# buggyyang/CDC_compression

Hardware: AMD Instinct MI355X
Metric: decoded images/sec at 256x256, 500-step x-param (higher is better)
Workload: dtype f32 (f16x2 split products)

## Files before the change

cdc_compression_amd/_lib.py:

```python
import ctypes
import os
import subprocess

import numpy as np

_HERE = os.path.dirname(os.path.abspath(__file__))
LIB_PATH = os.environ.get("CDC_HIP_LIB") or os.path.join(_HERE, "libcdc_hip.so")

CDC_MEM_HOST, CDC_MEM_DEVICE = 0, 1
CDC_PRED_X, CDC_PRED_NOISE, CDC_PRED_NOISE_XTREE, CDC_PRED_V = 0, 1, 2, 3
CDC_CLIP_NONE, CDC_CLIP_ALL, CDC_CLIP_HALF = 0, 1, 2
CDC_MAX_LEVELS = 8
CDC_ELEM_F32, CDC_ELEM_U8 = 0, 1
CDC_FILL_EDGE, CDC_FILL_ZERO = 0, 1
CDC_METRIC_PSNR, CDC_METRIC_MSSSIM = 1, 2
CDC_TRACE_X0, CDC_TRACE_XT, CDC_TRACE_U8 = 1, 2, 4

_f = ctypes.POINTER(ctypes.c_float)
_i = ctypes.c_int
_vp = ctypes.c_void_p


class UnetConfig(ctypes.Structure):
    _fields_ = [("dim", ctypes.c_int32), ("channels", ctypes.c_int32),
# ... 138 lines not shown
    L.cdc_prof_name.argtypes = [_i]
    L.cdc_prof_name.restype = ctypes.c_char_p
    L.cdc_prof_get.argtypes = [H, _i, ctypes.POINTER(ctypes.c_double),
                               ctypes.POINTER(ctypes.c_int64), ctypes.POINTER(ctypes.c_double),
                               ctypes.POINTER(ctypes.c_double)]
    L.cdc_prof_reset.argtypes = [H]
    L.cdc_prof_num_ops.argtypes = [H]
    L.cdc_prof_op.argtypes = [H, _i, ctypes.POINTER(ctypes.c_char_p), ctypes.POINTER(ctypes.c_double),
                              ctypes.POINTER(ctypes.c_int64), ctypes.POINTER(ctypes.c_double)]
    L.cdc_op_conv2d.argtypes = [H, _vp, _vp, _vp, _vp] + [_i] * 9 + [_vp, _vp, _i, _vp, _vp]
    L.cdc_op_conv_transpose2d.argtypes = [H, _vp, _vp, _vp, _vp] + [_i] * 5
    L.cdc_op_chan_layernorm.argtypes = [H, _vp, _vp, _vp, _vp, _i, _i, _i]
    L.cdc_op_chan_layernorm_ex.argtypes = [H, _vp, _i, _vp, _vp, _i, _vp, _vp, _i, _vp, _vp, _vp, _i, _i, _i]
    L.cdc_op_ln_form.argtypes = [H, _i, _i, _i, _i, _i] + [ctypes.POINTER(_i)] * 4
    L.cdc_op_sum_slices.argtypes = [H, _vp, _i, _vp, _i, ctypes.c_longlong]
    L.cdc_op_linear_attention.argtypes = [H] + [_vp] * 7 + [_i] * 4
    L.cdc_op_stress.argtypes = [H, _i]
    L.cdc_op_stress_result.argtypes = [H, ctypes.POINTER(ctypes.c_int64), ctypes.POINTER(ctypes.c_int64)]
    L.cdc_probe_mfma_f16.argtypes = [_i, _i, _i, ctypes.POINTER(ctypes.c_double)]
    L.cdc_probe_hbm_copy.argtypes = [_i, ctypes.c_size_t, _i, ctypes.POINTER(ctypes.c_double)]
    _lib = L
    return L


EXPORTS = ["cdc_create", "cdc_destroy", "cdc_last_error", "cdc_version", "cdc_num_tensors",
           "cdc_tensor_info", "cdc_load_tensor", "cdc_finalize_weights", "cdc_unet_forward",
           "cdc_set_schedule", "cdc_ddim_step", "cdc_decode", "cdc_prof_enable",
           "cdc_prof_num_classes", "cdc_prof_name", "cdc_prof_get", "cdc_prof_reset",
           "cdc_op_conv2d", "cdc_op_conv_transpose2d", "cdc_op_chan_layernorm",
           "cdc_op_linear_attention", "cdc_ctxdec_create", "cdc_ctxdec_decode", "cdc_hyperdec_create",
           "cdc_hyperdec_decode", "cdc_dequantize", "cdc_bpp", "cdc_encoder_create",
           "cdc_encoder_encode", "cdc_set_arith", "cdc_get_arith", "cdc_unet_tap", "cdc_prof_num_ops", "cdc_prof_op",
           "cdc_entropy_encode", "cdc_entropy_peek", "cdc_entropy_set_limit", "cdc_entropy_decode", "cdc_get_range_faults",
           "cdc_get_nonfinite_results", "cdc_set_schedule_v", "cdc_probe_mfma_f16", "cdc_probe_hbm_copy",
           "cdc_op_stress", "cdc_op_stress_result", "cdc_enable_vbr", "cdc_set_bitrate_scale", "cdc_entropy_peek_bitrate_scale",
           "cdc_padded_size", "cdc_frame_pad", "cdc_frame_crop", "cdc_entropy_set_image_scale", "cdc_entropy_encode_image",
           "cdc_entropy_peek_image_size", "cdc_decode_seeded", "cdc_randn", "cdc_randn_host", "cdc_philox4x32_10",
           "cdc_distortion", "cdc_lpips_create", "cdc_lpips", "cdc_simple_encoder_create", "cdc_simple_ctxdec_create", "cdc_op_gdn",
           "cdc_op_gdn_workgroups", "cdc_op_chan_layernorm_ex", "cdc_op_ln_form", "cdc_op_sum_slices",
           "cdc_set_solver", "cdc_decode_solver", "cdc_solver_step", "cdc_op_solver_update", "cdc_op_ddim_update",
           "cdc_repeat_images", "cdc_decode_samples", "cdc_sample_moments", "cdc_sample_select",
           "cdc_set_trace", "cdc_trace_info", "cdc_trace_read", "cdc_op_trace_tap"]


def handle_status(handle):
    if handle is None:
        return {"arith": None, "range_faults": 0, "nonfinite_results": 0}
    L = lib()
    return {"arith": int(L.cdc_get_arith(handle)), "range_faults": int(L.cdc_get_range_faults(handle)),
            "nonfinite_results": int(L.cdc_get_nonfinite_results(handle))}


def check(handle, rc):
    if rc != 0:
        msg = lib().cdc_last_error(handle)
        msg = msg.decode() if msg else ""
        if "must be multiples of" in msg:
# ... 90 lines not shown
```

cdc_compression_amd/csrc/cdc_internal.h:

```cpp
#pragma once
#include <stdio.h>
#include <string.h>
#include <stdlib.h>
#include <hip/hip_runtime.h>
#include <map>
#include <mutex>
#include <utility>
#include <stdint.h>

#include <string>
#include <vector>

#include "conv_args.h"

extern "C" char **environ;

namespace cdc {

typedef void (*conv_kernel_fn)(const ConvArgs);
conv_kernel_fn conv_lookup_a(int MB, int NPW, int lnmode);
conv_kernel_fn conv_lookup_b(int MB, int NPW, int lnmode);
conv_kernel_fn conv_lookup_c(int MB, int NPW, int lnmode);
conv_kernel_fn conv_lookup_split(int MB, int NPW);
conv_kernel_fn conv_lookup_split2(int MB, int NPW, int lnmode, int xu = 1);
// ... 23 lines not shown
    int stride = 1;
    int uf = 0;
    int cop = 0;
    int tz = 1;
};
struct PfPlan {
    int MB, NPW, WM, WP, ring, tiles_x, tiles_y, groups; size_t lds_bytes; int lin = 0;
    int x16 = 0;
    int pf3_epv = 0, pf3_G = 0, pf3_iters = 0;
};
bool pf_make_plan(const PfShape &s, PfPlan *plan);
hipError_t pf_launch(PfArgs a, const PfPlan &plan, int B, int nz, hipStream_t st);
bool pf3_make_plan(const PfArgs &a, int B, int nz, PfPlan *plan);
hipError_t pf3_launch(PfArgs a, const PfPlan &plan, int B, hipStream_t st);
int device_cus();
struct WsPlan { int W, NPB, stride, waves, tiles, groups; size_t lds_bytes; };
struct WsArgs;
bool ws_make_plan(int Cin, int C0, int Cout, int H, int W, int B, int stride, WsPlan *plan);
hipError_t ws_launch(WsArgs a, const WsPlan &plan, hipStream_t st);
struct Ws1Plan { int NPB, waves, tiles, groups; size_t lds_bytes; };
struct Ws1Args;
bool ws1_make_plan(int Cin, int C0, int Cout, int HW, int B, bool per_image_w, Ws1Plan *plan);
hipError_t ws1_launch(Ws1Args a, const Ws1Plan &plan, hipStream_t st);
bool pw_make_plan(const PfShape &s, PfPlan *plan);
hipError_t pw_launch(PfArgs a, const PfPlan &plan, int B, hipStream_t st);
hipError_t pf_pack_launch(const float *src, long long src_bs, void *dst, long long dst_bs, int C, int H, int W, int B,
                          hipStream_t st);
hipError_t c4_pack_launch(const float *src, long long src_bs, float *dst, int C, long long HW, int B, hipStream_t st);
hipError_t pf_unpack_launch(const void *src, long long src_bs, float *dst, long long dst_bs, int C, int H, int W, int B, hipStream_t st);

// ... 228 lines not shown
```

cdc_compression_amd/csrc/cdc_planner.hip:

```cpp
#include "cdc_state.h"

namespace cdcapi {

constexpr int kKsTarget = 1024;

struct Builder {
    cdc_handle *h;
    int B;
    std::vector<void *> *pool;
    int rc = CDC_OK;
    int planB = 0;
    int pb() const { return planB > 0 ? planB : B; }
    std::vector<Op> *cur = nullptr;

    void emit(Op op) {
        op.id = (int)h->op_ms.size();
        h->op_ms.push_back(0); h->op_n.push_back(0); h->op_flops.push_back(op.flops);
        const bool hoisted = cur == &h->pre_ops;
        char buf[160];
        std::visit([&](const auto &payload) { op_label(payload, buf, sizeof buf, hoisted); }, op.p);
        if (hoisted && !strstr(buf, " HOIST") && strlen(buf) + 7 < sizeof buf) strcat(buf, " HOIST");
        h->op_label.push_back(buf);
        (cur ? cur : &h->ops)->push_back(op);
    }
// ... 1493 lines not shown
int cdc_op_ln_form(cdc_handle *h, int B, int C, int HW, int nparts, int aligned16, int *kind, int *width, int *np, int *img_major) {
    if (!h) return CDC_ERR_INVALID;
    if (B < 1 || C < 1 || HW < 1 || nparts < 1) return fail(h, CDC_ERR_INVALID, "cdc_op_ln_form: B = %d, C = %d, HW = %d, nparts = %d", B, C, HW, nparts);
    if (nparts > 1 && C > 384) return fail(h, CDC_ERR_INVALID, "cdc_op_ln_form: %d split-K slices over %d > 384 channels", nparts, C);
    LnArgs a = {};
    a.C = C; a.HW = HW; a.nparts = nparts; a.part_stride = (long long)B * C * HW;
    a.in = reinterpret_cast<const float *>((uintptr_t)(aligned16 ? 16 : 4));
    const LnForm f = ln_form(a, B);
    if (kind) *kind = f.kind;
    if (width) *width = f.width;
    if (np) *np = f.np;
    if (img_major) *img_major = f.img_major;
    return CDC_OK;
}

int cdc_op_linear_attention(cdc_handle *h, const float *x, const float *norm_g, const float *norm_b,
                            const float *w_qkv, const float *w_out, const float *b_out, float *y, int B,
                            int C, int H, int W) {
    return with_range_guard(h, [&] { return op_linear_attention_impl(h, x, norm_g, norm_b, w_qkv, w_out, b_out, y, B, C, H, W); });
}

static int op_gdn_impl(cdc_handle *h, const float *x, const float *beta, const float *gamma, float *y, int B, int C, int HW, int inverse) {
    int rc = op_ready(h);
    if (rc) return rc;
    if (!x || !beta || !gamma || !y || B < 1 || HW < 1) return fail(h, CDC_ERR_INVALID, "null/invalid argument");
    if (!gdn_supported(C)) return fail(h, CDC_ERR_UNSUPPORTED, "GDN over %d channels: the kernel takes multiples of 16 from 16 to 256", C);
    OpScope sc(h);
    Builder bd{h, B, &sc.pool};
    std::vector<float> br((size_t)C), gr((size_t)C * C);
    gdn_reparam(beta, gamma, C, br.data(), gr.data());
// ... 48 lines not shown
```

cdc_compression_amd/csrc/conv_args.h:

```cpp
#pragma once
#include <stdint.h>

namespace cdc {

constexpr int kWaveSize = 64;
constexpr int kXS = 20;

struct ConvArgs {
    const float *src0, *src1;
    long long src0_bs, src1_bs;
    int uf_c, uf_pad;
    unsigned uf_magic;
    int C0, Cin;
    int H, W;
    const float *ln_mean, *ln_rstd;
    const float *ln_g, *ln_b;
    const float *wp;
    long long w_bs, w_zs;
    const unsigned short *wsp;
    long long wsp_zs;
    long long wsp_bs;
    float acc_scale;
    int tg;
    int ipw, B;
// ... 73 lines not shown
    long long resid1_bs;
    int resid_c0;
    const void *resid_pf;
    long long rpf_bs, rpf_ps;
    int rpf_ys, rpf_zoff;
    float *stat_mean, *stat_rstd;
    const float *res3_w, *res3_x;
    long long res3_bs;
    const float *x0, *x1;
    long long x0_bs, x1_bs;
    const float *pre_mean, *pre_rstd;
    long long w_bs;
    int lin;
    int dbg;
    int *fault;
#ifdef CDC_TIMELINE
    unsigned long long *tl;
#endif
};

constexpr int kPfXS = 12;

struct ConvPlan {
    int MB, NPW, WN;
    int groups;
    int KC, nchunk;
    int lognbw, tiles_x, tiles_y, PH, PW;
    int xvec, xshift[4];
    size_t lds_bytes;
    int lnmode;
// ... 10 lines not shown
```

cdc_compression_amd/csrc/conv_inst_p.hip:

```cpp
#include <algorithm>
#include <map>
#include <string>
#include <vector>
#include <stdlib.h>

#include "cdc_internal.h"
#include "conv_pf_kernel.h"

namespace cdc {

template <int KH, int KW>
static pf_kernel_fn pf_lookup_k(int MB, int NPW, int WM, int WP) {
    if (MB == 2 && NPW == 2 && WM == 1 && WP == 4) return conv_pf_kernel<2, 2, 1, 4, KH, KW>;
    if (MB == 2 && NPW == 2 && WM == 2 && WP == 2) return conv_pf_kernel<2, 2, 2, 2, KH, KW>;
    if (MB == 2 && NPW == 2 && WM == 2 && WP == 4) return conv_pf_kernel<2, 2, 2, 4, KH, KW>;
    if (MB == 3 && NPW == 2 && WM == 2 && WP == 4) return conv_pf_kernel<3, 2, 2, 4, KH, KW>;
    if (MB == 3 && NPW == 1 && WM == 2 && WP == 4 && KH == 3) return conv_pf_kernel<3, 1, 2, 4, KH, KW>;
    if (MB == 2 && NPW == 2 && WM == 4 && WP == 2) return conv_pf_kernel<2, 2, 4, 2, KH, KW>;
    return nullptr;
}
static pf_kernel_fn pf_lookup_s2(int MB, int NPW, int WM, int WP) {
    if (MB == 2 && NPW == 1 && WM == 1 && WP == 4) return conv_pf_kernel<2, 1, 1, 4, 3, 3, 2>;
    if (MB == 2 && NPW == 2 && WM == 2 && WP == 2) return conv_pf_kernel<2, 2, 2, 2, 3, 3, 2>;
    if (MB == 3 && NPW == 1 && WM == 2 && WP == 4) return conv_pf_kernel<3, 1, 2, 4, 3, 3, 2>;
// ... 148 lines not shown
            p->groups = s.Cout / COPT;
            p->lds_bytes = std::max(patch + ring * wst, sizeof(float) * (size_t)(4 * COPT + 2 * c.WM * c.WP * c.NPW * 32));
        }
    }
    return best >= 0;
}

hipError_t pf_launch(PfArgs a, const PfPlan &p, int B, int nz, hipStream_t st) {
    if (p.pf3_epv) return pf3_launch(a, p, B, st);
    pf_kernel_fn fn = pf_lookup(p.MB, p.NPW, p.WM, p.WP, a.KH, a.KW, a.stride == 2 ? 2 : 1, a.tz == 4 ? 4 : 1);
    if (!fn) return hipErrorInvalidValue;
    if (a.tz == 4) nz = 1;
    a.lognbw = 5;
    a.dbg = 0;
    a.tiles_x = p.tiles_x; a.tiles_y = p.tiles_y; a.B = B; a.ring = p.ring;
    if (hipError_t e = ensure_dynamic_lds((const void *)fn, p.lds_bytes); e != hipSuccess) return e;
    dim3 grid((unsigned)(p.tiles_x * p.tiles_y * B), (unsigned)p.groups, (unsigned)nz);
    a.xcd_remap = (grid.x % 8 == 0 && grid.x >= 64) ? 1 : 0;
#ifdef CDC_TIMELINE
    static unsigned long long *tl_dev = nullptr;
    static std::map<std::string, int> seen;
    const size_t tl_wgs = (size_t)grid.x * grid.y * grid.z;
    char key[96];
    snprintf(key, sizeof key, "%dx%d s%d tz%d %d->%d out %dx%d", a.KH, a.KW, a.stride == 2 ? 2 : 1, a.tz == 4 ? 4 : 1, a.Cin, a.Cout, a.Ho, a.Wo);
    a.tl = nullptr;
    if (tl_wgs <= (1u << 18) && seen[key]++ < 3) {
        if (!tl_dev) hipMalloc(&tl_dev, sizeof(unsigned long long) * 16 * (1u << 18));
        hipMemsetAsync(tl_dev, 0, sizeof(unsigned long long) * 16 * tl_wgs, st);
        a.tl = tl_dev;
    }
#endif
    hipLaunchKernelGGL(fn, grid, dim3(64 * p.WM * p.WP), p.lds_bytes, st, a);
#ifdef CDC_TIMELINE
    if (a.tl) {
        hipStreamSynchronize(st);
        std::vector<unsigned long long> h(16 * tl_wgs);
        hipMemcpy(h.data(), tl_dev, h.size() * 8, hipMemcpyDeviceToHost);
        unsigned long long t0 = ~0ull, t1 = 0;
        double cat[7] = {0}, life = 0;
        std::map<unsigned long long, int> per_cu;
        std::vector<unsigned long long> starts;
        for (size_t w = 0; w < tl_wgs; ++w) {
            const unsigned long long *r = &h[w * 16];
            for (int c = 0; c < 7; ++c) cat[c] += (double)r[c];
            t0 = std::min(t0, r[7]); t1 = std::max(t1, r[8]);
            life += (double)(r[8] - r[7]);
            per_cu[(r[10] & 0xf) << 32 | (r[9] & 0xffff00)]++;
// ... 89 lines not shown
```

cdc_compression_amd/csrc/conv_pf_kernel.h:

```cpp
#pragma once
#include <type_traits>

#include "conv_split_kernel.h"

namespace cdc {


#ifndef CDC_DMA_WAIT_MARGIN
#define CDC_DMA_WAIT_MARGIN 1
#endif
#ifdef CDC_DMA_WAIT_ALL
constexpr int kVmWaitMask = 0;
#else
constexpr int kVmWaitMask = ~0;
#endif
template <int N> __device__ __forceinline__ void vm_wait() { asm volatile("s_waitcnt vmcnt(%0)" ::"n"(N & kVmWaitMask) : "memory"); }

__device__ __forceinline__ void dma16(unsigned voff, const void *sbase, unsigned lds_byte) {
    asm volatile("s_mov_b32 m0, %2\n\ts_nop 0\n\tglobal_load_lds_dwordx4 %0, %1" ::"v"(voff), "s"(sbase), "s"(lds_byte)
                 : "memory");
}

template <int N, class F> __device__ __forceinline__ void static_for(F &&f) {
    if constexpr (N > 0) {
// ... 27 lines not shown
#define CDC_PF_S2_TPS 3
#endif
#ifndef CDC_PF_TZ_MINB
#define CDC_PF_TZ_MINB 2
#endif
#ifndef CDC_PF_TZ_TPS
#define CDC_PF_TZ_TPS 2
#endif
__host__ __device__ constexpr int pf_tps(int MB, int NPW, int WM, int WP, int KH, int KW, int STR = 1, int TZ = 1) {
    if (TZ == 4) return (CDC_PF_TZ_TPS > 1 && pf_ring_tps(MB, NPW, WM, WP, KH, KW, STR, CDC_PF_TZ_TPS, TZ) >= 3) ? CDC_PF_TZ_TPS : 1;
    return (STR == 2 && CDC_PF_S2_TPS > 1 && pf_ring_tps(MB, NPW, WM, WP, KH, KW, STR, CDC_PF_S2_TPS) >= 3) ? CDC_PF_S2_TPS : 1;
}
__host__ __device__ constexpr int pf_ring(int MB, int NPW, int WM, int WP, int KH, int KW, int STR = 1, int TZ = 1) {
    return pf_ring_tps(MB, NPW, WM, WP, KH, KW, STR, pf_tps(MB, NPW, WM, WP, KH, KW, STR, TZ), TZ);
}
#ifndef CDC_PF_ABLATE
#define CDC_PF_ABLATE 0
#endif

template <int MB, int NPW, int WM, int WP, int KH, int KW, int STR = 1, int TZ = 1, int UF = 0>
__global__ void __launch_bounds__(64 * WM * WP, (KH == 1 && KW == 7) ? 3 : STR == 2 ? 1 : ((WM * WP == 8 || MB * NPW * TZ <= 4 || (TZ == 4 && MB * NPW <= 2 && CDC_PF_TZ_MINB == 2)) ? 2 : 1)) conv_pf_kernel(const PfArgs P) {
    constexpr int NW = WM * WP, NT = 64 * NW, COPT = WM * MB * 32;
    static_assert(COPT % 64 == 0 || COPT == 32, "a weight DMA instruction (64 units) must stay inside one (plane, k-half) row");
    static_assert(TZ == 1 || (TZ == 4 && KH == 2 && KW == 2 && STR == 1), "fused phases: the 2x2 phase form of the 4x4 transposed convolution");
    constexpr int NB = TZ * NPW;
    constexpr bool ACC2 = pf_acc2(MB, NB);
    constexpr int NPL = ACC2 ? 2 : 3, ROWS = 2 * NPL;
    constexpr int WI = (ROWS * COPT + 63) / 64;
    constexpr int NWV = NW - 2;
    constexpr int NWW = (WI + NWV - 1) / NWV;
    constexpr int TAPZ = KH * KW, TAPS = TAPZ * TZ;
    constexpr int NBW = 32, NBH = 1;
    constexpr int TH = WP * NPW * NBH;
    constexpr int PH = TZ == 4 ? TH + 2 : (TH - 1) * STR + KH, PW = TZ == 4 ? NBW + 2 : (NBW - 1) * STR + KW, PLANE = PH * PW;
    constexpr int NE = (PW + 1) / 2;
// ... 20 lines not shown
        unsigned hw_; asm volatile("s_getreg_b32 %0, hwreg(HW_REG_HW_ID)" : "=s"(hw_)); r_[9] = hw_; \
        unsigned xcc_; asm volatile("s_getreg_b32 %0, hwreg(HW_REG_XCC_ID)" : "=s"(xcc_)); r_[10] = xcc_; } } while (0)
#else
#define PFTL(c) do { } while (0)
#define PFTL_END() do { } while (0)
#endif
    const int tid = threadIdx.x, lane = tid & 63;
    const int wave = __builtin_amdgcn_readfirstlane(tid >> 6);
    const int wm = wave / WP, wp = wave % WP;
    const bool patch_wave = wave >= NWV;
    const int pwi = wave - NWV;
    const int z = blockIdx.z, cog = blockIdx.y;
    unsigned bid0 = blockIdx.x;
    if (P.xcd_remap) bid0 = (bid0 & 7) * (gridDim.x >> 3) + (bid0 >> 3);
    int bid = (int)bid0;
    const int tx = bid % P.tiles_x;
    bid /= P.tiles_x;
    const int ty = bid % P.tiles_y;
    const int b = bid / P.tiles_y;
    const int oy0 = ty * TH, ox0 = tx * NBW;
    const int S = P.nchunk * SPC;
    constexpr int R = pf_ring(MB, NPW, WM, WP, KH, KW, STR, TZ);
    static_assert(R >= 3, "no room for a weight ring");
    const unsigned lds0 = __builtin_amdgcn_readfirstlane((unsigned)(size_t)(const __attribute__((address_space(3))) uint4 *)smem_u);
    const unsigned wl_lds = lds0 + (unsigned)(NPB * PST) * 16u;

    const int Hp = P.H + 2, Wp = P.W + 2;
    const int iy0 = oy0 * STR - P.pad_y[z] + 1, ix0 = ox0 * STR - P.pad_x[z] + 1;
    unsigned xoff[KX];
#pragma unroll
    for (int i = 0; i < KX; ++i) {
        int e = (2 * i + (pwi & 1)) * 64 + lane;
        if (e >= NX) e = 0;
        const int q = e / PLANE, rem = e - q * PLANE;
        const int r = rem / PW, cp = rem - r * PW;
        const int c = STR == 2 ? (cp < NE ? 2 * cp : 2 * (cp - NE) + 1) : cp;
        const int iy = min(max(iy0 + r, 0), Hp - 1), ix = min(max(ix0 + c, 0), Wp - 1);
        xoff[i] = (unsigned)((q * Hp + iy) * Wp + ix) * 16u;
    }
    const long long cg_bytes = (long long)4 * Hp * Wp * 16;
    const char *s0 = reinterpret_cast<const char *>(P.src0) + (size_t)b * P.src0_bs * 16;
    const char *s1 = P.src1 ? reinterpret_cast<const char *>(P.src1) + (size_t)b * P.src1_bs * 16 : nullptr;
    const int c0_chunks = P.C0 >> 4;
    constexpr int ISSUE_TAPS = TAPS >= 9 ? 6 : (TAPS == 7 ? 5 : (TAPS >= 4 ? 2 : 1));
    constexpr int PER = (KX + ISSUE_TAPS - 1) / ISSUE_TAPS;
    auto issue_patch = [&](int chunk, auto tc) {
        constexpr int t = decltype(tc)::value;
        const char *base = chunk < c0_chunks ? s0 + (long long)chunk * cg_bytes : s1 + (long long)(chunk - c0_chunks) * cg_bytes;
        int pb = chunk;
        if constexpr (NPB == 2) pb &= 1; else pb %= 3;
        const unsigned dst = lds0 + (unsigned)(pb * PST) * 16u + (unsigned)(pwi & 1) * 1024u;
#pragma unroll
        for (int i = 0; i < KX; ++i)
            if (t < 0 || i / PER == t)
// ... 18 lines not shown
    const char *wptr = wsrc;
    int tw = 0, sw = 0;
    auto issue_w = [&]() {
        const unsigned dst = wl_lds + (unsigned)(sw * WST) * 16u;
#pragma unroll
        for (int q = 0; q < TPS; ++q)
#pragma unroll
            for (int k = 0; k < NWW; ++k) dma16(wvo[k], wptr + q * w_dt, dst + (unsigned)(q * TAPW) * 16u + wdo[k]);
        tw += TPS;
        if (tw == TAPS) { tw = 0; wptr += w_dc; }
        else if (TZ > 1 && (tw % TAPZ) == 0) wptr += w_dz;
        else wptr += TPS * w_dt;
        if (++sw == R) sw = 0;
    };

    f32x16 acc[MB][NB], acc2[ACC2 ? MB : 1][ACC2 ? NB : 1];
#pragma unroll
    for (int m = 0; m < MB; ++m)
#pragma unroll
        for (int n = 0; n < NB; ++n)
#pragma unroll
            for (int r = 0; r < 16; ++r) {
                acc[m][n][r] = 0.f;
                if constexpr (ACC2) acc2[m][n][r] = 0.f;
            }

    const int half = lane >> 5, j = lane & 31;
    const int pr = 0, pc = j;
    const uint4 *a_base = smem_u + NPB * PST + half * COPT + wm * MB * 32 + j;
    const uint4 *b_base = smem_u + (half * 2) * PLANE + (wp * NPW * STR) * PW + j;

// ... 33 lines not shown
#pragma unroll
            for (int term = 0; term < 3; ++term) {
                constexpr int PA[3] = {1, 2, 0};
                constexpr int PB[3] = {0, 1, 0};
#pragma unroll
                for (int m = 0; m < MB; ++m)
#pragma unroll
                    for (int n = 0; n < NPW; ++n)
                        acc[m][q0 + n] = __builtin_amdgcn_mfma_f32_32x32x16_f16(A[PA[term] % NPL][m], Bv[PB[term]][n], acc[m][q0 + n], 0, 0, 0);
            }
        }
    };

    PFTL(0);
    if constexpr (UF != 0) {
        if (!patch_wave)
            for (int q = 0; q < R - 1 && q < S; ++q) issue_w();
        constexpr int XW = NBW + 6;
        float *xs = reinterpret_cast<float *>(smem_u + NPB * PST + R * WST);
        {
            constexpr int NS = (UF * PH * XW + NT - 1) / NT;
            float sv[NS];
#pragma unroll
            for (int k = 0; k < NS; ++k) {
                const int i = tid + k * NT;
                const int ci = i / (PH * XW), rem = i - ci * (PH * XW), r = rem / XW, cc = rem - r * XW;
                const int iy = oy0 - 3 + r, ix = ox0 - 3 + cc;
                sv[k] = (i < UF * PH * XW && iy >= 0 && iy < P.H && ix >= 0 && ix < P.W) ? P.x0[(size_t)b * P.x0_bs + ((size_t)ci * P.H + iy) * P.W + ix] : 0.f;
            }
#pragma unroll
            for (int k = 0; k < NS; ++k)
                if (tid + k * NT < UF * PH * XW) xs[tid + k * NT] = sv[k];
// ... 5 lines not shown
#pragma unroll
            for (int ch = 0; ch < 32; ++ch) {
                if (ch < 7 * UF) split2h(xs[((ch % UF) * PH + r) * XW + c + ch / UF], hq[ch], lq[ch]);
                else { hq[ch] = (_Float16)0.f; lq[ch] = (_Float16)0.f; }
            }
#pragma unroll
            for (int q = 0; q < 4; ++q) {
                f16x8 hv, lv;
#pragma unroll
                for (int t = 0; t < 8; ++t) { hv[t] = hq[8 * q + t]; lv[t] = lq[8 * q + t]; }
                uint4 *pbuf = smem_u + (q >> 1) * PST + ((q & 1) * 2) * PLANE + px;
                pbuf[0] = __builtin_bit_cast(uint4, hv);
                pbuf[PLANE] = __builtin_bit_cast(uint4, lv);
            }
        }
    } else if (patch_wave) {
        for (int c = 0; c < LA && c < P.nchunk; ++c) issue_patch(c, std::integral_constant<int, -1>{});
    } else {
        for (int q = 0; q < R - 1 && q < S; ++q) issue_w();
    }
    PFTL(1);
    dma_wait();
    __builtin_amdgcn_s_barrier();
    PFTL(2);
    OpsA A0, A1;
    OpsB B0, B1;
    fetch(std::integral_constant<int, 0>{}, b_base, a_base, A0, B0);
    int rem = S - 1;
    int sn = 0;
    auto tap = [&](auto tc, auto tailc, int chunk, const uint4 *xb_cur, const uint4 *xb_nxt, OpsA &Ac, OpsB &Bc, OpsA &An,
                   OpsB &Bn) {
        constexpr int t = decltype(tc)::value;
        constexpr bool TAIL = decltype(tailc)::value;
        constexpr bool SEND = (t % TPS) == TPS - 1;
// ... 59 lines not shown
    } else {
        int chunk = 0;
        for (; chunk + 1 < n_main; chunk += 2) {
            chunk_body(P0{}, std::false_type{}, chunk);
            chunk_body(P1{}, std::false_type{}, chunk + 1);
        }
        for (; chunk + 1 < P.nchunk; chunk += 2) {
            chunk_body(P0{}, std::true_type{}, chunk);
            chunk_body(P1{}, std::true_type{}, chunk + 1);
        }
        if (chunk < P.nchunk) chunk_body(P0{}, std::true_type{}, chunk);
    }

    __builtin_amdgcn_s_barrier();
    PFTL(3);
    if (CDC_PF_ABLATE && (P.dbg & 256)) { PFTL_END(); return; }
    float *ep = reinterpret_cast<float *>(smem_u);
    float *red = ep + 4 * COPT;
    for (int i = tid; i < COPT; i += NT) {
        const int co = cog * COPT + i;
        const bool ok = co < P.Cout;
        ep[i] = (ok && P.bias) ? P.bias[co] : 0.f;
        ep[COPT + i] = (ok && P.ep_g) ? P.ep_g[co] : 0.f;
        ep[2 * COPT + i] = (ok && P.ep_b) ? P.ep_b[co] : 0.f;
        ep[3 * COPT + i] = (ok && P.shift) ? P.shift[(size_t)b * P.shift_bs + co] : 0.f;
    }
    __syncthreads();
    PFTL(4);
    const float inv_c = 1.0f / (float)P.Cout;
    const int cobase = cog * COPT + wm * MB * 32;
    const float *epl = ep + wm * MB * 32 + 4 * half;
    const bool ch_ok = cobase + MB * 32 <= P.Cout || COPT == 32;
    const int nvalid = P.Cout - cobase;
    if constexpr (TZ == 4) {
        if (!P.pre_add && !P.resid && !P.resid_pf && !P.res3_w && !P.relu && !P.shift && !P.stat_mean && (WM == 1 || !P.ep_g)) {
            static_assert(!ACC2, "fused phases: one accumulator set");
#pragma unroll
            for (int py = 0; py < 2; ++py)
#pragma unroll
                for (int n = 0; n < NPW; ++n) {
                    const int q0 = (py * 2) * NPW + n, q1 = q0 + NPW;
                    const int oy = oy0 + (wp * NPW + n) * NBH + pr, ox = ox0 + pc;
// ... 78 lines not shown
                                    const uint2 sh = half ? a0 : a1, sl = half ? c0 : c1;
                                    uint2 rh, rl;
                                    rh.x = __shfl_xor(sh.x, 32); rh.y = __shfl_xor(sh.y, 32);
                                    rl.x = __shfl_xor(sl.x, 32); rl.y = __shfl_xor(sl.y, 32);
                                    const uint4 uh = half ? make_uint4(rh.x, rh.y, a1.x, a1.y) : make_uint4(a0.x, a0.y, rh.x, rh.y);
                                    const uint4 ul = half ? make_uint4(rl.x, rl.y, c1.x, c1.y) : make_uint4(c0.x, c0.y, rl.x, rl.y);
                                    uint4 *pu = reinterpret_cast<uint4 *>(P.out_pf) + u0 + (long long)((cobase >> 3) + m * 4 + g) * 2 * P.pf_ps;
                                    pu[0] = uh;
                                    pu[P.pf_ps] = ul;
                                }
                        }
                    }
                    __builtin_amdgcn_sched_barrier(0);
                }
            PFTL(6);
            PFTL_END();
            return;
        }
    }
    float mean_v[NB], rinv_v[NB];
    bool valid_v[NB];
    unsigned pix_v[NB];
#pragma unroll
    for (int n = 0; n < NB; ++n) {
        const int oy = oy0 + (wp * NPW + n % NPW) * NBH + pr, ox = ox0 + pc;
        const int zn = TZ == 4 ? n / NPW : z;
        valid_v[n] = (oy < P.Ho) && (ox < P.Wo) && ch_ok;
        pix_v[n] = (unsigned)(oy * P.out_ys + ox * P.out_xs + P.out_zoff[zn]);
        const float *eq = epl;
#pragma unroll
        for (int m = 0; m < MB; ++m)
#pragma unroll
// ... 197 lines not shown
                            const uint2 a0 = __builtin_bit_cast(uint2, hv0), a1 = __builtin_bit_cast(uint2, hv1);
                            const uint2 c0 = __builtin_bit_cast(uint2, lv0), c1 = __builtin_bit_cast(uint2, lv1);
                            const uint2 sh = half ? a0 : a1, sl = half ? c0 : c1;
                            uint2 rh, rl;
                            rh.x = __shfl_xor(sh.x, 32); rh.y = __shfl_xor(sh.y, 32);
                            rl.x = __shfl_xor(sl.x, 32); rl.y = __shfl_xor(sl.y, 32);
                            const uint4 uh = half ? make_uint4(rh.x, rh.y, a1.x, a1.y) : make_uint4(a0.x, a0.y, rh.x, rh.y);
                            const uint4 ul = half ? make_uint4(rl.x, rl.y, c1.x, c1.y) : make_uint4(c0.x, c0.y, rl.x, rl.y);
                            uint4 *pu = reinterpret_cast<uint4 *>(P.out_pf) + u0 + (long long)((cobase >> 3) + m * 4 + g) * 2 * P.pf_ps;
                            pu[0] = uh;
                            pu[P.pf_ps] = ul;
                        }
                }
            }
        PFTL(6);
        PFTL_END();
        return;
    }
#pragma unroll
    for (int n = 0; n < NB; ++n) {
        if (!valid_v[n] || (CDC_PF_ABLATE && (P.dbg & 16))) continue;
        if (P.out) {
            float *op = P.out + (size_t)b * P.out_bs + pix_v[n] + (size_t)(cobase + 4 * half) * P.out_cs;
#pragma unroll
            for (int m = 0; m < MB; ++m)
#pragma unroll
                for (int r = 0; r < 16; ++r) {
                    const int ci = m * 32 + (r & 3) + 8 * (r >> 2);
                    if (COPT != 32 || ci + 4 * half < nvalid) op[(size_t)ci * P.out_cs] = acc[m][n][r];
                }
        }
        if (P.out_pf) {
            const int oy = oy0 + (wp * NPW + n % NPW) * NBH + pr, ox = ox0 + pc;
            const long long u0 = (long long)b * P.pf_bs + (long long)oy * P.pf_ys + (long long)ox * P.pf_xs + P.pf_zoff[TZ == 4 ? n / NPW : z];
#pragma unroll
            for (int m = 0; m < MB; ++m)
                pf_store_block(reinterpret_cast<uint4 *>(P.out_pf), u0 + (long long)((cobase >> 3) + m * 4) * 2 * P.pf_ps, P.pf_ps, half, acc[m][n]);
        }
    }
    PFTL(6);
    PFTL_END();
}

typedef void (*pf_kernel_fn)(const PfArgs);

}
```

cdc_compression_amd/ops.py:

```python
import ctypes

import numpy as np

from . import _lib


def _c(a):
    return None if a is None else np.ascontiguousarray(a, dtype=np.float32)


def _p(a):
    return None if a is None else a.ctypes.data


class Ops:
    def __init__(self, device=0):
        def config():
            cfg = _lib.UnetConfig()
            cfg.dim, cfg.channels, cfg.context_channels, cfg.out_dim = 32, 3, 3, 3
            cfg.n_dim_mults = 1
            cfg.dim_mults[0] = 1
            cfg.n_context_dim_mults = 1
            cfg.context_dim_mults[0] = 1
            return cfg
# ... 94 lines not shown
        return y

    def gdn(self, x, beta, gamma, inverse=False):
        x, beta, gamma = _c(x), _c(beta).reshape(-1), _c(gamma)
        B, C, H, W = x.shape
        if beta.shape != (C,) or gamma.shape != (C, C):
            raise ValueError(f"beta {beta.shape} / gamma {gamma.shape} do not belong to {C} channels")
        y = np.empty_like(x)
        _lib.check(self._h, _lib.lib().cdc_op_gdn(self._h, _p(x), _p(beta), _p(gamma), _p(y), B, C, H * W, int(bool(inverse))))
        return y

    def gdn_workgroups(self, B, HW):
        per_image, tiles = ctypes.c_int(), ctypes.c_int()
        _lib.check(self._h, _lib.lib().cdc_op_gdn_workgroups(self._h, int(B), int(HW), ctypes.byref(per_image), ctypes.byref(tiles)))
        return per_image.value, tiles.value
```

include/cdc_hip.h:

```cpp
#ifndef CDC_HIP_H
#define CDC_HIP_H

#include <stddef.h>
#include <stdint.h>

#ifdef __cplusplus
extern "C" {
#endif

typedef struct cdc_handle cdc_handle;

typedef enum {
    CDC_OK = 0,
    CDC_ERR_INVALID = -1,
    CDC_ERR_STATE = -2,
    CDC_ERR_HIP = -3,
    CDC_ERR_UNSUPPORTED = -4,
    CDC_ERR_NOMEM = -5
} cdc_status;

enum { CDC_MEM_HOST = 0, CDC_MEM_DEVICE = 1 };
enum { CDC_PRED_X = 0, CDC_PRED_NOISE = 1, CDC_PRED_NOISE_XTREE = 2, CDC_PRED_V = 3 };
enum { CDC_CLIP_NONE = 0, CDC_CLIP_ALL = 1, CDC_CLIP_HALF = 2 };
enum { CDC_MAX_LEVELS = 8 };
// ... 183 lines not shown
int cdc_prof_num_ops(cdc_handle *h);
int cdc_prof_op(cdc_handle *h, int idx, const char **label, double *ms, int64_t *launches, double *flops);


int cdc_op_conv2d(cdc_handle *h, const float *x, const float *w, const float *bias, float *y,
                  int B, int Cin, int H, int W, int Cout, int KH, int KW, int stride, int pad,
                  const float *ln_g, const float *ln_b, int relu, const float *shift,
                  const float *resid);
int cdc_op_conv_transpose2d(cdc_handle *h, const float *x, const float *w, const float *bias,
                            float *y, int B, int Cin, int H, int W, int Cout);
int cdc_op_chan_layernorm(cdc_handle *h, const float *x, const float *g, const float *b, float *y,
                          int B, int C, int HW);
int cdc_op_chan_layernorm_ex(cdc_handle *h, const float *x, int nparts, const float *g, const float *b, int relu, const float *shift,
                             const float *resid, int in_place, float *y, float *stat_mean, float *stat_rstd, int B, int C, int HW);
int cdc_op_ln_form(cdc_handle *h, int B, int C, int HW, int nparts, int aligned16, int *kind, int *width, int *np, int *img_major);
int cdc_op_sum_slices(cdc_handle *h, const float *x, int parts, float *y, int B, long long n);
int cdc_op_gdn(cdc_handle *h, const float *x, const float *beta, const float *gamma, float *y, int B, int C, int HW, int inverse);
int cdc_op_gdn_workgroups(cdc_handle *h, int B, int HW, int *per_image, int *tiles);
int cdc_op_linear_attention(cdc_handle *h, const float *x, const float *norm_g,
                            const float *norm_b, const float *w_qkv, const float *w_out,
                            const float *b_out, float *y, int B, int C, int H, int W);

int cdc_op_stress(cdc_handle *h, int repeats);
int cdc_op_stress_result(cdc_handle *h, int64_t *launches, int64_t *differing);

#ifdef __cplusplus
}
#endif
#endif
```

Before: 5.271.

## Add persistent walking form of stride-2 3x3 pf conv kernel

Adds a WALK template variant of the pf conv kernel in which each workgroup processes a contiguous range of tiles in a loop, sized to the number of resident slots. While the current tile's epilogue runs, it prefetches the next tile's patches and weights, and it reuses the bias and LN epilogue parameters across tiles. Only stride-2 3x3 shapes with two specific MB/NPW/WM/WP configs use it. It aims to cut per-workgroup launch, prologue and pipeline-fill cost, in exchange for more LDS use, a more complex kernel and possible load imbalance across workgroups.

```diff
diff --git a/cdc_compression_amd/_lib.py b/cdc_compression_amd/_lib.py
--- a/cdc_compression_amd/_lib.py
+++ b/cdc_compression_amd/_lib.py
@@ -176,6 +176,11 @@
     L.cdc_op_chan_layernorm_ex.argtypes = [H, _vp, _i, _vp, _vp, _i, _vp, _vp, _i, _vp, _vp, _vp, _i, _i, _i]
     L.cdc_op_ln_form.argtypes = [H, _i, _i, _i, _i, _i] + [ctypes.POINTER(_i)] * 4
     L.cdc_op_sum_slices.argtypes = [H, _vp, _i, _vp, _i, ctypes.c_longlong]
+    L.cdc_pf_walk_ranges.argtypes = [_i, _i, _i, _vp]
+    L.cdc_pf_walk_tile.argtypes = [_i, _i, _i, _i]
+    L.cdc_pf_walk_wgs.argtypes = [_i, _i]
+    L.cdc_pf_walk_launches.argtypes = []
+    L.cdc_pf_walk_launches.restype = ctypes.c_longlong
     L.cdc_op_linear_attention.argtypes = [H] + [_vp] * 7 + [_i] * 4
     L.cdc_op_stress.argtypes = [H, _i]
     L.cdc_op_stress_result.argtypes = [H, ctypes.POINTER(ctypes.c_int64), ctypes.POINTER(ctypes.c_int64)]
@@ -202,7 +207,8 @@
            "cdc_op_gdn_workgroups", "cdc_op_chan_layernorm_ex", "cdc_op_ln_form", "cdc_op_sum_slices",
            "cdc_set_solver", "cdc_decode_solver", "cdc_solver_step", "cdc_op_solver_update", "cdc_op_ddim_update",
            "cdc_repeat_images", "cdc_decode_samples", "cdc_sample_moments", "cdc_sample_select",
-           "cdc_set_trace", "cdc_trace_info", "cdc_trace_read", "cdc_op_trace_tap"]
+           "cdc_set_trace", "cdc_trace_info", "cdc_trace_read", "cdc_op_trace_tap",
+           "cdc_pf_walk_ranges", "cdc_pf_walk_tile", "cdc_pf_walk_wgs", "cdc_pf_walk_launches"]
 
 
 def handle_status(handle):
diff --git a/cdc_compression_amd/csrc/cdc_internal.h b/cdc_compression_amd/csrc/cdc_internal.h
--- a/cdc_compression_amd/csrc/cdc_internal.h
+++ b/cdc_compression_amd/csrc/cdc_internal.h
@@ -3,6 +3,8 @@
 #include <string.h>
 #include <stdlib.h>
 #include <hip/hip_runtime.h>
+#include <algorithm>
+#include <atomic>
 #include <map>
 #include <mutex>
 #include <utility>
@@ -61,6 +63,23 @@
 bool pf3_make_plan(const PfArgs &a, int B, int nz, PfPlan *plan);
 hipError_t pf3_launch(PfArgs a, const PfPlan &plan, int B, hipStream_t st);
 int device_cus();
+typedef void (*pf_kernel_fn_t)(const PfArgs);
+pf_kernel_fn_t pf_walk_lookup(int MB, int NPW, int WM, int WP, int KH, int KW, int stride, int tz);
+extern std::atomic<long long> g_pf_walk_launches;
+inline int pf_walk_wgs(int tiles, int slots) {
+    const int g = std::max(1, std::min(tiles, slots));
+    return g >= 64 ? g & ~7 : g;
+}
+inline int pf_walk_first(int tiles, int wgs, int wg) { return wg * (tiles / wgs) + std::min(wg, tiles % wgs); }
+inline int pf_walk_tile(int t, int tiles_x, int tiles_y, int col_major) {
+    const int per = tiles_x * tiles_y, b = t / per, ti = t % per;
+    return col_major ? b * per + (ti % tiles_y) * tiles_x + ti / tiles_y : t;
+}
+inline int pf_walk_slots(int KH, int KW, int stride, size_t lds_bytes, int yz) {
+    int per_cu = stride == 2 ? 1 : ((KH == 1 && KW == 7) ? 3 : 2);
+    if (lds_bytes) per_cu = std::max(1, std::min(per_cu, (int)(160 * 1024 / lds_bytes)));
+    return std::max(1, device_cus() * per_cu / std::max(1, yz));
+}
 struct WsPlan { int W, NPB, stride, waves, tiles, groups; size_t lds_bytes; };
 struct WsArgs;
 bool ws_make_plan(int Cin, int C0, int Cout, int H, int W, int B, int stride, WsPlan *plan);
diff --git a/cdc_compression_amd/csrc/cdc_planner.hip b/cdc_compression_amd/csrc/cdc_planner.hip
--- a/cdc_compression_amd/csrc/cdc_planner.hip
+++ b/cdc_compression_amd/csrc/cdc_planner.hip
@@ -1531,6 +1531,22 @@
     return CDC_OK;
 }
 
+int cdc_pf_walk_ranges(int tiles, int wgs_lo, int wgs_hi, int *first) {
+    if (tiles < 1 || wgs_lo < 1 || wgs_hi < wgs_lo || !first) return CDC_ERR_INVALID;
+    for (int wgs = wgs_lo; wgs <= wgs_hi; ++wgs)
+        for (int wg = 0; wg <= wgs; ++wg) *first++ = pf_walk_first(tiles, wgs, wg);
+    return CDC_OK;
+}
+
+int cdc_pf_walk_tile(int t, int tiles_x, int tiles_y, int col_major) {
+    if (t < 0 || tiles_x < 1 || tiles_y < 1) return CDC_ERR_INVALID;
+    return pf_walk_tile(t, tiles_x, tiles_y, col_major);
+}
+
+int cdc_pf_walk_wgs(int tiles, int slots) { return (tiles < 1 || slots < 1) ? CDC_ERR_INVALID : pf_walk_wgs(tiles, slots); }
+
+long long cdc_pf_walk_launches(void) { return g_pf_walk_launches.load(); }
+
 int cdc_op_linear_attention(cdc_handle *h, const float *x, const float *norm_g, const float *norm_b,
                             const float *w_qkv, const float *w_out, const float *b_out, float *y, int B,
                             int C, int H, int W) {
diff --git a/cdc_compression_amd/csrc/conv_args.h b/cdc_compression_amd/csrc/conv_args.h
--- a/cdc_compression_amd/csrc/conv_args.h
+++ b/cdc_compression_amd/csrc/conv_args.h
@@ -111,6 +111,7 @@
     int lin;
     int dbg;
     int *fault;
+    int walk_q, walk_r;
 #ifdef CDC_TIMELINE
     unsigned long long *tl;
 #endif
diff --git a/cdc_compression_amd/csrc/conv_inst_p.hip b/cdc_compression_amd/csrc/conv_inst_p.hip
--- a/cdc_compression_amd/csrc/conv_inst_p.hip
+++ b/cdc_compression_amd/csrc/conv_inst_p.hip
@@ -186,8 +186,24 @@
     a.lognbw = 5;
     a.dbg = 0;
     a.tiles_x = p.tiles_x; a.tiles_y = p.tiles_y; a.B = B; a.ring = p.ring;
-    if (hipError_t e = ensure_dynamic_lds((const void *)fn, p.lds_bytes); e != hipSuccess) return e;
     dim3 grid((unsigned)(p.tiles_x * p.tiles_y * B), (unsigned)p.groups, (unsigned)nz);
+    size_t lds_bytes = p.lds_bytes;
+    if (pf_kernel_fn wfn = dev_env("CDC_PF_NO_WALK") ? nullptr : pf_walk_lookup(p.MB, p.NPW, p.WM, p.WP, a.KH, a.KW, a.stride == 2 ? 2 : 1, a.tz == 4 ? 4 : 1)) {
+        const int tiles = (int)grid.x;
+        const size_t wl = pf_walk_lds_bytes(p.MB, p.NPW, p.WM, p.WP, a.KH, a.KW, a.stride == 2 ? 2 : 1, a.tz == 4 ? 4 : 1);
+        int wgs = pf_walk_wgs(tiles, pf_walk_slots(a.KH, a.KW, a.stride == 2 ? 2 : 1, wl, p.groups * nz));
+        if (const char *cap = dev_env("CDC_PF_MAX_WGS"))
+            if (atoi(cap) > 0) wgs = pf_walk_wgs(tiles, atoi(cap));
+        if (wl && wgs < tiles) {
+            fn = wfn;
+            lds_bytes = wl;
+            grid.x = (unsigned)wgs;
+            a.walk_q = tiles / wgs; a.walk_r = tiles % wgs;
+            a.lin = a.KH > 1 ? 1 : 0;
+            ++g_pf_walk_launches;
+        }
+    }
+    if (hipError_t e = ensure_dynamic_lds((const void *)fn, lds_bytes); e != hipSuccess) return e;
     a.xcd_remap = (grid.x % 8 == 0 && grid.x >= 64) ? 1 : 0;
 #ifdef CDC_TIMELINE
     static unsigned long long *tl_dev = nullptr;
@@ -202,7 +218,7 @@
         a.tl = tl_dev;
     }
 #endif
-    hipLaunchKernelGGL(fn, grid, dim3(64 * p.WM * p.WP), p.lds_bytes, st, a);
+    hipLaunchKernelGGL(fn, grid, dim3(64 * p.WM * p.WP), lds_bytes, st, a);
 #ifdef CDC_TIMELINE
     if (a.tl) {
         hipStreamSynchronize(st);
diff --git a/cdc_compression_amd/csrc/conv_inst_v.hip b/cdc_compression_amd/csrc/conv_inst_v.hip
--- /dev/null
+++ b/cdc_compression_amd/csrc/conv_inst_v.hip
@@ -0,0 +1,17 @@
+#include "cdc_internal.h"
+#include "conv_pf_kernel.h"
+
+namespace cdc {
+
+std::atomic<long long> g_pf_walk_launches{0};
+
+pf_kernel_fn_t pf_walk_lookup(int MB, int NPW, int WM, int WP, int KH, int KW, int stride, int tz) {
+    if (stride == 2 && tz == 1 && KH == 3 && KW == 3) {
+        if (MB == 2 && NPW == 1 && WM == 1 && WP == 4) return conv_pf_kernel<2, 1, 1, 4, 3, 3, 2, 1, 0, 1>;
+        if (MB == 2 && NPW == 2 && WM == 2 && WP == 2) return conv_pf_kernel<2, 2, 2, 2, 3, 3, 2, 1, 0, 1>;
+        return nullptr;
+    }
+    return nullptr;
+}
+
+}
diff --git a/cdc_compression_amd/csrc/conv_pf_kernel.h b/cdc_compression_amd/csrc/conv_pf_kernel.h
--- a/cdc_compression_amd/csrc/conv_pf_kernel.h
+++ b/cdc_compression_amd/csrc/conv_pf_kernel.h
@@ -65,11 +65,24 @@
 __host__ __device__ constexpr int pf_ring(int MB, int NPW, int WM, int WP, int KH, int KW, int STR = 1, int TZ = 1) {
     return pf_ring_tps(MB, NPW, WM, WP, KH, KW, STR, pf_tps(MB, NPW, WM, WP, KH, KW, STR, TZ), TZ);
 }
+__host__ __device__ constexpr size_t pf_walk_ep_bytes(int MB, int NPW, int WM, int WP, int TZ = 1) {
+    return sizeof(float) * (size_t)(4 * WM * MB * 32 + (WM > 1 ? 2 * WM * WP * TZ * NPW * 32 : 0));
+}
+__host__ __device__ constexpr size_t pf_walk_ep_offset(int MB, int NPW, int WM, int WP, int KH, int KW, int STR = 1, int TZ = 1) {
+    return (size_t)pf_patch_bufs(KH, KW, STR) * pf_patch_units(NPW, WP, KH, KW, STR, TZ) * 16 +
+           (size_t)pf_ring(MB, NPW, WM, WP, KH, KW, STR, TZ) * pf_tps(MB, NPW, WM, WP, KH, KW, STR, TZ) * pf_rows(MB, TZ * NPW) * WM * MB * 32 * 16 +
+           ((KH == 7 && KW == 1) ? (size_t)pf_uf_stage_floats(NPW, WP) * 4 : 0);
+}
+__host__ __device__ constexpr size_t pf_walk_lds_bytes(int MB, int NPW, int WM, int WP, int KH, int KW, int STR = 1, int TZ = 1) {
+    const size_t limit = (WM * WP == 8 || STR == 2) ? 160 * 1024 : ((KH == 1 && KW == 7) ? 160 * 1024 / 3 : 80 * 1024);
+    const size_t used = pf_walk_ep_offset(MB, NPW, WM, WP, KH, KW, STR, TZ) + pf_walk_ep_bytes(MB, NPW, WM, WP, TZ);
+    return (pf_ring(MB, NPW, WM, WP, KH, KW, STR, TZ) >= 3 && used <= limit) ? used : 0;
+}
 #ifndef CDC_PF_ABLATE
 #define CDC_PF_ABLATE 0
 #endif
 
-template <int MB, int NPW, int WM, int WP, int KH, int KW, int STR = 1, int TZ = 1, int UF = 0>
+template <int MB, int NPW, int WM, int WP, int KH, int KW, int STR = 1, int TZ = 1, int UF = 0, int WALK = 0>
 __global__ void __launch_bounds__(64 * WM * WP, (KH == 1 && KW == 7) ? 3 : STR == 2 ? 1 : ((WM * WP == 8 || MB * NPW * TZ <= 4 || (TZ == 4 && MB * NPW <= 2 && CDC_PF_TZ_MINB == 2)) ? 2 : 1)) conv_pf_kernel(const PfArgs P) {
     constexpr int NW = WM * WP, NT = 64 * NW, COPT = WM * MB * 32;
     static_assert(COPT % 64 == 0 || COPT == 32, "a weight DMA instruction (64 units) must stay inside one (plane, k-half) row");
@@ -120,11 +133,23 @@
     unsigned bid0 = blockIdx.x;
     if (P.xcd_remap) bid0 = (bid0 & 7) * (gridDim.x >> 3) + (bid0 >> 3);
     int bid = (int)bid0;
-    const int tx = bid % P.tiles_x;
-    bid /= P.tiles_x;
-    const int ty = bid % P.tiles_y;
-    const int b = bid / P.tiles_y;
-    const int oy0 = ty * TH, ox0 = tx * NBW;
+    int tx, ty, b;
+    int left = 1;
+    if constexpr (WALK) {
+        left = P.walk_q + (bid < P.walk_r ? 1 : 0);
+        if (left == 0) return;
+        const int t = bid * P.walk_q + min(bid, P.walk_r), per = P.tiles_x * P.tiles_y;
+        b = t / per;
+        const int ti = t - b * per;
+        if (P.lin) { tx = ti / P.tiles_y; ty = ti - tx * P.tiles_y; }
+        else { ty = ti / P.tiles_x; tx = ti - ty * P.tiles_x; }
+    } else {
+        tx = bid % P.tiles_x;
+        bid /= P.tiles_x;
+        ty = bid % P.tiles_y;
+        b = bid / P.tiles_y;
+    }
+    int oy0 = ty * TH, ox0 = tx * NBW;
     const int S = P.nchunk * SPC;
     constexpr int R = pf_ring(MB, NPW, WM, WP, KH, KW, STR, TZ);
     static_assert(R >= 3, "no room for a weight ring");
@@ -132,18 +157,21 @@
     const unsigned wl_lds = lds0 + (unsigned)(NPB * PST) * 16u;
 
     const int Hp = P.H + 2, Wp = P.W + 2;
-    const int iy0 = oy0 * STR - P.pad_y[z] + 1, ix0 = ox0 * STR - P.pad_x[z] + 1;
+    int iy0 = oy0 * STR - P.pad_y[z] + 1, ix0 = ox0 * STR - P.pad_x[z] + 1;
     unsigned xoff[KX];
-#pragma unroll
-    for (int i = 0; i < KX; ++i) {
-        int e = (2 * i + (pwi & 1)) * 64 + lane;
-        if (e >= NX) e = 0;
-        const int q = e / PLANE, rem = e - q * PLANE;
-        const int r = rem / PW, cp = rem - r * PW;
-        const int c = STR == 2 ? (cp < NE ? 2 * cp : 2 * (cp - NE) + 1) : cp;
-        const int iy = min(max(iy0 + r, 0), Hp - 1), ix = min(max(ix0 + c, 0), Wp - 1);
-        xoff[i] = (unsigned)((q * Hp + iy) * Wp + ix) * 16u;
-    }
+    auto set_xoff = [&]() {
+#pragma unroll
+        for (int i = 0; i < KX; ++i) {
+            int e = (2 * i + (pwi & 1)) * 64 + lane;
+            if (e >= NX) e = 0;
+            const int q = e / PLANE, rem = e - q * PLANE;
+            const int r = rem / PW, cp = rem - r * PW;
+            const int c = STR == 2 ? (cp < NE ? 2 * cp : 2 * (cp - NE) + 1) : cp;
+            const int iy = min(max(iy0 + r, 0), Hp - 1), ix = min(max(ix0 + c, 0), Wp - 1);
+            xoff[i] = (unsigned)((q * Hp + iy) * Wp + ix) * 16u;
+        }
+    };
+    set_xoff();
     const long long cg_bytes = (long long)4 * Hp * Wp * 16;
     const char *s0 = reinterpret_cast<const char *>(P.src0) + (size_t)b * P.src0_bs * 16;
     const char *s1 = P.src1 ? reinterpret_cast<const char *>(P.src1) + (size_t)b * P.src1_bs * 16 : nullptr;
@@ -192,7 +220,32 @@
         if (++sw == R) sw = 0;
     };
 
+    auto issue_first = [&]() {
+        if (UF == 0 && patch_wave) {
+            for (int c = 0; c < LA && c < P.nchunk; ++c) issue_patch(c, std::integral_constant<int, -1>{});
+        } else if (!patch_wave) {
+            for (int q = 0; q < R - 1 && q < S; ++q) issue_w();
+        }
+    };
+    static_assert(!WALK || pf_walk_lds_bytes(MB, NPW, WM, WP, KH, KW, STR, TZ) != 0, "the shape has no LDS left for a walking form");
+    constexpr size_t EPO = WALK ? pf_walk_ep_offset(MB, NPW, WM, WP, KH, KW, STR, TZ) / sizeof(float) : 0;
+    float *ep = reinterpret_cast<float *>(smem_u) + EPO;
+    float *red = ep + 4 * COPT;
+    auto ep_args = [&]() -> decltype(auto) {
+        if constexpr (WALK) {
+            typedef const __attribute__((address_space(4))) PfArgs PfArgsK;
+            PfArgsK *kp = (PfArgsK *)__builtin_amdgcn_kernarg_segment_ptr();
+            asm volatile("" : "+s"(kp));
+            return (*kp);
+        } else {
+            return (P);
+        }
+    };
+    int b_ep = -1;
+    bool fetched = false;
+
     f32x16 acc[MB][NB], acc2[ACC2 ? MB : 1][ACC2 ? NB : 1];
+    for (;;) {
 #pragma unroll
     for (int m = 0; m < MB; ++m)
 #pragma unroll
@@ -256,8 +309,7 @@
 
     PFTL(0);
     if constexpr (UF != 0) {
-        if (!patch_wave)
-            for (int q = 0; q < R - 1 && q < S; ++q) issue_w();
+        if (!(WALK && fetched)) issue_first();
         constexpr int XW = NBW + 6;
         float *xs = reinterpret_cast<float *>(smem_u + NPB * PST + R * WST);
         {
@@ -293,10 +345,8 @@
                 pbuf[PLANE] = __builtin_bit_cast(uint4, lv);
             }
         }
-    } else if (patch_wave) {
-        for (int c = 0; c < LA && c < P.nchunk; ++c) issue_patch(c, std::integral_constant<int, -1>{});
-    } else {
-        for (int q = 0; q < R - 1 && q < S; ++q) issue_w();
+    } else if (!(WALK && fetched)) {
+        issue_first();
     }
     PFTL(1);
     dma_wait();
@@ -386,18 +436,55 @@
 
     __builtin_amdgcn_s_barrier();
     PFTL(3);
-    if (CDC_PF_ABLATE && (P.dbg & 256)) { PFTL_END(); return; }
-    float *ep = reinterpret_cast<float *>(smem_u);
-    float *red = ep + 4 * COPT;
-    for (int i = tid; i < COPT; i += NT) {
-        const int co = cog * COPT + i;
-        const bool ok = co < P.Cout;
-        ep[i] = (ok && P.bias) ? P.bias[co] : 0.f;
-        ep[COPT + i] = (ok && P.ep_g) ? P.ep_g[co] : 0.f;
-        ep[2 * COPT + i] = (ok && P.ep_b) ? P.ep_b[co] : 0.f;
-        ep[3 * COPT + i] = (ok && P.shift) ? P.shift[(size_t)b * P.shift_bs + co] : 0.f;
-    }
-    __syncthreads();
+    if constexpr (WALK) {
+        fetched = left > 1;
+        if (fetched) {
+            int nb = b, nty = ty, ntx = tx;
+            if (P.lin) {
+                if (++nty == P.tiles_y) { nty = 0; if (++ntx == P.tiles_x) { ntx = 0; ++nb; } }
+            } else {
+                if (++ntx == P.tiles_x) { ntx = 0; if (++nty == P.tiles_y) { nty = 0; ++nb; } }
+            }
+            const int niy0 = nty * TH * STR - P.pad_y[z] + 1, nix0 = ntx * NBW * STR - P.pad_x[z] + 1;
+            const bool in_cur = iy0 >= 0 && iy0 + PH <= Hp && ix0 >= 0 && ix0 + PW <= Wp;
+            const bool in_nxt = niy0 >= 0 && niy0 + PH <= Hp && nix0 >= 0 && nix0 + PW <= Wp;
+            const unsigned delta = (unsigned)(((niy0 - iy0) * Wp + (nix0 - ix0)) * 16);
+            iy0 = niy0; ix0 = nix0;
+            if (UF != 0) {
+            } else if (in_cur && in_nxt) {
+#pragma unroll
+                for (int i = 0; i < KX; ++i) xoff[i] += delta;
+            } else {
+                set_xoff();
+            }
+            if (nb != b) {
+                s0 = reinterpret_cast<const char *>(P.src0) + (size_t)nb * P.src0_bs * 16;
+                s1 = P.src1 ? reinterpret_cast<const char *>(P.src1) + (size_t)nb * P.src1_bs * 16 : nullptr;
+            }
+            wptr = wsrc; tw = 0; sw = 0;
+            issue_first();
+        }
+    }
+    do {
+    const auto &P = ep_args();
+    int lane_e = lane, wave_e = wave;
+    if constexpr (WALK) asm volatile("" : "+v"(lane_e), "+s"(wave_e));
+    const int half = lane_e >> 5, j = lane_e & 31, pc = j, wm = wave_e / WP, wp = wave_e % WP;
+    if (CDC_PF_ABLATE && (P.dbg & 256)) break;
+    if (!WALK || b_ep < 0 || (P.shift && b != b_ep)) {
+        for (int i = tid; i < COPT; i += NT) {
+            const int co = cog * COPT + i;
+            const bool ok = co < P.Cout;
+            if (!WALK || b_ep < 0) {
+                ep[i] = (ok && P.bias) ? P.bias[co] : 0.f;
+                ep[COPT + i] = (ok && P.ep_g) ? P.ep_g[co] : 0.f;
+                ep[2 * COPT + i] = (ok && P.ep_b) ? P.ep_b[co] : 0.f;
+            }
+            ep[3 * COPT + i] = (ok && P.shift) ? P.shift[(size_t)b * P.shift_bs + co] : 0.f;
+        }
+        b_ep = b;
+        __syncthreads();
+    }
     PFTL(4);
     const float inv_c = 1.0f / (float)P.Cout;
     const int cobase = cog * COPT + wm * MB * 32;
@@ -506,8 +593,7 @@
                     __builtin_amdgcn_sched_barrier(0);
                 }
             PFTL(6);
-            PFTL_END();
-            return;
+            break;
         }
     }
     float mean_v[NB], rinv_v[NB];
@@ -735,8 +821,7 @@
                 }
             }
         PFTL(6);
-        PFTL_END();
-        return;
+        break;
     }
 #pragma unroll
     for (int n = 0; n < NB; ++n) {
@@ -760,6 +845,15 @@
         }
     }
     PFTL(6);
+    } while (0);
+    if (!WALK || --left == 0) break;
+    if (P.lin) {
+        if (++ty == P.tiles_y) { ty = 0; if (++tx == P.tiles_x) { tx = 0; ++b; } }
+    } else {
+        if (++tx == P.tiles_x) { tx = 0; if (++ty == P.tiles_y) { ty = 0; ++b; } }
+    }
+    oy0 = ty * TH; ox0 = tx * NBW;
+    }
     PFTL_END();
 }
 
diff --git a/cdc_compression_amd/ops.py b/cdc_compression_amd/ops.py
--- a/cdc_compression_amd/ops.py
+++ b/cdc_compression_amd/ops.py
@@ -132,3 +132,32 @@
         per_image, tiles = ctypes.c_int(), ctypes.c_int()
         _lib.check(self._h, _lib.lib().cdc_op_gdn_workgroups(self._h, int(B), int(HW), ctypes.byref(per_image), ctypes.byref(tiles)))
         return per_image.value, tiles.value
+
+
+def pf_walk_wgs(tiles, slots):
+    g = max(1, min(int(tiles), int(slots)))
+    return g & ~7 if g >= 64 else g
+
+
+def pf_walk_first(tiles, wgs):
+    q, r = divmod(int(tiles), int(wgs))
+    wg = np.arange(int(wgs) + 1, dtype=np.int64)
+    return wg * q + np.minimum(wg, r)
+
+
+def pf_walk_tile(t, tiles_x, tiles_y, col_major):
+    per = tiles_x * tiles_y
+    b, ti = divmod(int(t), per)
+    return b * per + (ti % tiles_y) * tiles_x + ti // tiles_y if col_major else int(t)
+
+
+def pf_walk_ranges_c(tiles, wgs_lo, wgs_hi):
+    out = np.empty(sum(g + 1 for g in range(int(wgs_lo), int(wgs_hi) + 1)), np.int32)
+    rc = _lib.lib().cdc_pf_walk_ranges(int(tiles), int(wgs_lo), int(wgs_hi), out.ctypes.data)
+    if rc != 0:
+        raise ValueError(f"cdc_pf_walk_ranges({tiles}, {wgs_lo}, {wgs_hi}) = {rc}")
+    return out
+
+
+def pf_walk_launches():
+    return int(_lib.lib().cdc_pf_walk_launches())
diff --git a/include/cdc_hip.h b/include/cdc_hip.h
--- a/include/cdc_hip.h
+++ b/include/cdc_hip.h
@@ -221,6 +221,10 @@
 int cdc_op_chan_layernorm_ex(cdc_handle *h, const float *x, int nparts, const float *g, const float *b, int relu, const float *shift,
                              const float *resid, int in_place, float *y, float *stat_mean, float *stat_rstd, int B, int C, int HW);
 int cdc_op_ln_form(cdc_handle *h, int B, int C, int HW, int nparts, int aligned16, int *kind, int *width, int *np, int *img_major);
+int cdc_pf_walk_ranges(int tiles, int wgs_lo, int wgs_hi, int *first);
+int cdc_pf_walk_tile(int t, int tiles_x, int tiles_y, int col_major);
+int cdc_pf_walk_wgs(int tiles, int slots);
+long long cdc_pf_walk_launches(void);
 int cdc_op_sum_slices(cdc_handle *h, const float *x, int parts, float *y, int B, long long n);
 int cdc_op_gdn(cdc_handle *h, const float *x, const float *beta, const float *gamma, float *y, int B, int C, int HW, int inverse);
 int cdc_op_gdn_workgroups(cdc_handle *h, int B, int HW, int *per_image, int *tiles);
```

After: 5.278 (median of 6 runs). No clear change (+0.1%).
